# ketanfatania/QMRI-PnP-Recon-POC

Measured on NVIDIA B200. Metric: ADMM slice-iterations/s (224x224x10 slices; step = 120-slice PnP-ADMM recon + T1/T2/PD matching), higher is better.
Workload: dtype f32 (x-update fp32 FFT; denoiser split-bf16 tcgen05, fp32 accumulate; matching fp32)

## Files before the change

### qmri-pnp-recon-poc_b200/csrc/conv_kernels.h

```cpp
#pragma once
#include <stddef.h>
#include <stdint.h>

struct qmri_ctx;

struct ConvParams {
    const float* in;
    const float* w;
    float* out;
    const float* res1;
    const float* res2;
    int S, H, W;
    int Cin, Cout;
    int relu;
    int mode;
    const uint16_t* in_hi = nullptr;
    const uint16_t* in_lo = nullptr;
    uint16_t* out_hi = nullptr;
    uint16_t* out_lo = nullptr;
};

struct HeadTailParams {
    const float* planar_in;
    const float* noise_map;
    float* planar_out;
    float* nhwc;
    const float* w;
    const float* minmax;
    int S, H, W, Cin;
    uint16_t* nhwc_hi = nullptr;
    uint16_t* nhwc_lo = nullptr;
};

enum { TC_CONV3X3 = 0, TC_DOWN2X2 = 1, TC_UP2X2 = 2 };
struct TcConvParams {
    uint16_t* out_hi;
    uint16_t* out_lo;
    const uint16_t* res1_hi;
    const uint16_t* res1_lo;
    const uint16_t* res2_hi;
    const uint16_t* res2_lo;
    int mode;
    int S, H, W;
    int Cin, Cout;
    int BW, BH, tiles_x, tiles_y;
    int relu;
    float* partial;
    int* tickets;
    const void* mapA_hi[4];
    const void* mapA_lo[4];
    const void* mapB_hi;
    const void* mapB_lo;
    const void* mapB_h2;
    const void* mapB_l2;
    const void* mapO_hi;
    const void* mapO_lo;
    const void* mapR_hi;
    const void* mapR_lo;
};

int conv3x3_fp32(qmri_ctx* ctx, const ConvParams& p);
int resample_fp32(qmri_ctx* ctx, const ConvParams& p);
int head_fp32(qmri_ctx* ctx, const HeadTailParams& p);
int tail_fp32(qmri_ctx* ctx, const HeadTailParams& p);
int head_pack_tc(qmri_ctx* ctx, const HeadTailParams& p);
int tail_unpack_tc(qmri_ctx* ctx, const HeadTailParams& p);
int tc_make_act_map(void* out_map, const void* base, int S, int H, int W, int C, int BW, int BH);
int tc_make_down_map(void* out_map, const void* base, int S, int H, int W, int C, int dy, int dx, int BW, int BH);
int tc_make_weight_map(void* out_map, const void* base, int K, int N, int BN);
int tc_tile_shape(int W, int H, int* BW, int* BH);
int tc_block_n(int Cout);
size_t tc_partial_elems(int sm_count);
size_t tc_ticket_count(int sm_count);
int conv_tc(qmri_ctx* ctx, const TcConvParams& p);
int tc_slab_tile_shape(int W, int H, int* BW, int* BH);
void tc_pair_weight_boxes(int Cout, int* rows_main, int* rows_h2);
int conv3x3_tc_pair(qmri_ctx* ctx, const TcConvParams& p);
bool conv64_swap_supported(int W, int H, int Cin, int Cout);
int conv64_swap(qmri_ctx* ctx, const TcConvParams& p, const uint16_t* w_hi, const uint16_t* w_lo);
int normalize_planar(qmri_ctx* ctx, const float* in, float* out, const float* minmax, size_t per_slice, int S, int undo);
```

### qmri-pnp-recon-poc_b200/csrc/conv_tc.cu

```cuda
#include <cuda.h>
#include <cuda_bf16.h>
#include <math.h>
#include <stdlib.h>
#include <string.h>
#include <time.h>
#include <unistd.h>

#include "common.cuh"
#include "conv_kernels.h"

namespace {

constexpr int TC_THREADS = 192;
constexpr int PAIR_THREADS = 224;
constexpr int TC_BM = 128;
constexpr int TC_BK = 64;
constexpr uint32_t A_TILE_BYTES = TC_BM * TC_BK * 2;

template <int BN>
struct TcCfg {
    static constexpr uint32_t B_TILE_BYTES = BN * TC_BK * 2;
    static constexpr uint32_t STAGE_BYTES = 2 * A_TILE_BYTES + 2 * B_TILE_BYTES;
    static constexpr int STAGES = (BN == 64) ? 4 : 3;
    static constexpr uint32_t TMEM_COLS = 2 * BN;
// ... 1794 lines not shown
#pragma unroll
                    for (int i = 0; i < 16; ++i) {
                        const int co = 16 * seg + i;
                        v[i] = tile[co * SW_N + 32 * q + ((lane + co) & 31)];
                    }
                    const size_t o = (((size_t)s * p.H + y) * p.W + x) * 64 + 16 * seg;
                    if (p.res1_hi) {
                        const uint4* gh = reinterpret_cast<const uint4*>(p.res1_hi + o);
                        const uint4* gl = reinterpret_cast<const uint4*>(p.res1_lo + o);
                        add_split8(v, gh[0], gl[0]);
                        add_split8(v + 8, gh[1], gl[1]);
                    }
                    if (p.res2_hi) {
                        const uint4* gh = reinterpret_cast<const uint4*>(p.res2_hi + o);
                        const uint4* gl = reinterpret_cast<const uint4*>(p.res2_lo + o);
                        add_split8(v, gh[0], gl[0]);
                        add_split8(v + 8, gh[1], gl[1]);
                    }
                    store_split16(p.out_hi + o, p.out_lo + o, v, p.relu);
                }
            }
        }
    }
    tc_fence_before();
    __syncthreads();
    if (warp == 1) {
        tc_fence_after();
        asm volatile("tcgen05.dealloc.cta_group::1.sync.aligned.b32 %0, %1;" ::"r"(tmem_base), "r"(512));
    }
}

bool conv64_swap_supported(int W, int H, int Cin, int Cout) { return Cin == 64 && Cout == 64 && W % SW_BW == 0 && H % SW_BH == 0; }
int conv64_swap(qmri_ctx* ctx, const TcConvParams& p, const uint16_t* w_hi, const uint16_t* w_lo) {
    if (!conv64_swap_supported(p.W, p.H, p.Cin, p.Cout)) return qmri_fail(QMRI_EINVAL, "conv64_swap: %d x %d, %d -> %d channels", p.W, p.H, p.Cin, p.Cout);
    if (!p.mapA_hi[0] || !p.mapA_lo[0] || !w_hi || !w_lo) return qmri_fail(QMRI_EINVAL, "conv64_swap: missing tensor map / weights");
    static bool configured_dev[QMRI_MAX_DEV] = {};
    bool& configured = configured_dev[qmri_dev_slot(ctx)];
    if (!configured) {
        QCUDA(cudaFuncSetAttribute(tc_conv64_swap_kernel, cudaFuncAttributeMaxDynamicSharedMemorySize, (int)SW_SMEM));
        configured = true;
    }
    SwapK k;
    k.out_hi = p.out_hi; k.out_lo = p.out_lo;
    k.res1_hi = p.res1_hi; k.res1_lo = p.res1_lo;
    k.res2_hi = p.res2_hi; k.res2_lo = p.res2_lo;
    k.w_hi = w_hi; k.w_lo = w_lo;
    k.S = p.S; k.H = p.H; k.W = p.W;
    k.tiles_x = p.W / SW_BW; k.tiles_y = p.H / SW_BH;
    k.relu = p.relu;
    const int ntiles = k.tiles_x * k.tiles_y * p.S;
    cudaLaunchConfig_t cfg = {};
    cfg.gridDim = dim3(ntiles < ctx->sm_count ? ntiles : ctx->sm_count);
    cfg.blockDim = dim3(TC_THREADS);
    cfg.dynamicSmemBytes = SW_SMEM;
    cfg.stream = ctx->stream;
    cudaLaunchAttribute attr[1];
    attr[0].id = cudaLaunchAttributeProgrammaticStreamSerialization;
    attr[0].val.programmaticStreamSerializationAllowed = tc_pdl_enabled() ? 1 : 0;
    cfg.attrs = attr;
    cfg.numAttrs = 1;
    QCUDA(cudaLaunchKernelEx(&cfg, tc_conv64_swap_kernel, *(const CUtensorMap*)p.mapA_hi[0], *(const CUtensorMap*)p.mapA_lo[0], (const SwapK)k));
    QLAUNCH_CHECK(ctx);
    return QMRI_OK;
}

int conv3x3_tc_pair(qmri_ctx* ctx, const TcConvParams& p) {
    if (p.Cin % TC_BK) return qmri_fail(QMRI_EINVAL, "conv3x3_tc_pair: Cin %% 64");
    if (p.Cout != 64 && p.Cout != 128 && p.Cout % 256) return qmri_fail(QMRI_EINVAL, "conv3x3_tc_pair: Cout %d", p.Cout);
    if (p.BW % 8 || p.BW * p.BH != TC_BM || (p.BH + 2) * p.BW * 128 > (int)PairCfg<256, 0>::A_PLANE)
        return qmri_fail(QMRI_EINVAL, "conv3x3_tc_pair: tile %d x %d not supported", p.BW, p.BH);
    if (!p.mapA_hi[0] || !p.mapA_lo[0] || !p.mapB_hi || !p.mapB_lo || !p.mapB_h2) return qmri_fail(QMRI_EINVAL, "conv3x3_tc_pair: missing tensor map");
    TcK k;
    k.out_hi = p.out_hi; k.out_lo = p.out_lo;
    k.res1_hi = p.res1_hi; k.res1_lo = p.res1_lo;
    k.res2_hi = p.res2_hi; k.res2_lo = p.res2_lo;
    k.partial = p.partial; k.tickets = p.tickets;
    k.S = p.S; k.H = p.H; k.W = p.W; k.Cin = p.Cin; k.Cout = p.Cout;
    k.BW = p.BW; k.BH = p.BH; k.tiles_x = p.tiles_x; k.tiles_y = p.tiles_y;
    k.relu = p.relu; k.nsplit = 1; k.trace = nullptr; k.cluster_splitk = 0; k.dual = 0; k.resw = 0; k.tma_out = 0; k.res_tma = 0; k.l2pf = 0; k.prof = nullptr;
    if (p.Cout == 64) return launch_pair<128, 1>(ctx, p, k);
    if (p.Cout == 128) return launch_pair<256, 1>(ctx, p, k);
    return launch_pair<256, 0>(ctx, p, k);
}
```

### qmri-pnp-recon-poc_b200/csrc/unetres.cu

```cuda
#include <stdlib.h>
#include <string.h>

#include <vector>

#include "common.cuh"
#include "conv_kernels.h"
#include "unetres.h"

static const int NC[4] = {64, 128, 256, 512};

namespace {

struct LayerDesc {
    int kind;
    int cin, cout;
};

std::vector<LayerDesc> layer_table(int in_nc) {
    std::vector<LayerDesc> L;
    L.push_back({3, in_nc, NC[0]});
    for (int lvl = 0; lvl < 3; ++lvl) {
        for (int i = 0; i < 8; ++i) L.push_back({0, NC[lvl], NC[lvl]});
        L.push_back({1, NC[lvl], NC[lvl + 1]});
    }
// ... 80 lines not shown

size_t unetres_weight_count(int in_nc, int layer) {
    auto L = layer_table(in_nc);
    const LayerDesc& d = L[layer];
    int k = (d.kind == 1 || d.kind == 2) ? 4 : 9;
    return (size_t)k * d.cin * d.cout;
}

int unetres_create(qmri_ctx* ctx, int in_nc, const float* const* weights, int n_weights, qmri_net** out) {
    if (!ctx || !weights || !out) return qmri_fail(QMRI_EINVAL, "qmri_unetres_load: null argument");
    if (in_nc != 10 && in_nc != 11)
        return qmri_fail(QMRI_EUNSUPPORTED, "UNetRes in_nc must be 10 (single_level) or 11 (multi_level), got %d", in_nc);
    if (n_weights != 64) return qmri_fail(QMRI_EINVAL, "UNetRes state_dict has 64 weight tensors, got %d", n_weights);
    DevSetter ds(ctx->device);
    qmri_net* net = new qmri_net();
    net->ctx = ctx;
    net->in_nc = in_nc;
    if (const char* e = getenv("QMRI_TC_PAIR")) net->tc_pair = atoi(e);
    auto L = layer_table(in_nc);
    std::vector<float> packed;
    for (int o = 0; o < 2; ++o) {
        net->w[o].assign(64, nullptr);
        for (int l = 0; l < 64; ++l) {
            if (!weights[l]) {
                unetres_free(net);
                return qmri_fail(QMRI_EINVAL, "qmri_unetres_load: weight tensor %d is null", l);
            }
            pack_layer(L[l], weights[l], o, packed);
            int r = dev_alloc(&net->w[o][l], packed.size());
            if (r) {
                unetres_free(net);
                return r;
            }
            cudaError_t e = cudaMemcpy(net->w[o][l], packed.data(), packed.size() * sizeof(float), cudaMemcpyHostToDevice);
            if (e != cudaSuccess) {
                unetres_free(net);
                return qmri_fail(QMRI_ECUDA, "weight upload failed: %s", cudaGetErrorString(e));
            }
        }
        net->wtc_hi[o].assign(64, nullptr);
        net->wtc_lo[o].assign(64, nullptr);
        net->wmap_hi[o].resize(64);
        net->wmap_lo[o].resize(64);
        net->wmapp_hi[o].resize(64);
        net->wmapp_lo[o].resize(64);
        net->wmapp_h2[o].resize(64);
        net->wmapp_l2[o].resize(64);
        std::vector<uint16_t> hi, lo;
        std::vector<float> wpad;
        for (int l = 0; l < 64 && net->tc_available; ++l) {
            LayerDesc dl = L[l];
            const float* wsrc = weights[l];
            if (dl.kind > 2) {
                wpad.assign((size_t)64 * 64 * 9, 0.f);
                for (int co = 0; co < dl.cout; ++co)
                    for (int ci = 0; ci < dl.cin; ++ci)
                        for (int t = 0; t < 9; ++t) wpad[((size_t)co * 64 + ci) * 9 + t] = weights[l][((size_t)co * dl.cin + ci) * 9 + t];
                dl = LayerDesc{0, 64, 64};
                wsrc = wpad.data();
            }
            pack_layer_tc(dl, wsrc, o, hi, lo);
            int r = dev_alloc(&net->wtc_hi[o][l], hi.size()) | dev_alloc(&net->wtc_lo[o][l], lo.size());
            if (r) {
                unetres_free(net);
                return r;
            }
            cudaMemcpy(net->wtc_hi[o][l], hi.data(), hi.size() * 2, cudaMemcpyHostToDevice);
            cudaMemcpy(net->wtc_lo[o][l], lo.data(), lo.size() * 2, cudaMemcpyHostToDevice);
            const int BN = tc_block_n(dl.cout);
            const int K = (dl.kind == 0 ? 9 : dl.kind == 1 ? 4 : 1) * dl.cin;
            const int N = (dl.kind == 2 ? 4 : 1) * dl.cout;
            r = tc_make_weight_map(&net->wmap_hi[o][l], net->wtc_hi[o][l], K, N, BN) |
                tc_make_weight_map(&net->wmap_lo[o][l], net->wtc_lo[o][l], K, N, BN);
            if (!r && dl.kind == 0) {
                int rows_main, rows_h2;
                tc_pair_weight_boxes(dl.cout, &rows_main, &rows_h2);
                r = tc_make_weight_map(&net->wmapp_hi[o][l], net->wtc_hi[o][l], K, N, rows_main) |
                    tc_make_weight_map(&net->wmapp_lo[o][l], net->wtc_lo[o][l], K, N, rows_main) |
                    tc_make_weight_map(&net->wmapp_h2[o][l], net->wtc_hi[o][l], K, N, rows_h2) |
                    tc_make_weight_map(&net->wmapp_l2[o][l], net->wtc_lo[o][l], K, N, rows_h2);
            }
            if (r) net->tc_available = false;
        }
    }
    if (net->tc_available) {
        const size_t np = tc_partial_elems(ctx->sm_count), nt = tc_ticket_count(ctx->sm_count);
        int r = dev_alloc(&net->tc_partial, np) | dev_alloc(&net->tc_tickets, nt);
        if (r) {
            unetres_free(net);
            return r;
        }
        cudaMemset(net->tc_tickets, 0, nt * sizeof(int));
    } else {
        net->precision = 0;
    }
    *out = net;
    return QMRI_OK;
}

void unetres_free(qmri_net* net) {
    if (!net) return;
    DevSetter ds(net->ctx->device);
    for (int o = 0; o < 2; ++o) {
        for (float* p : net->w[o])
            if (p) cudaFree(p);
        for (uint16_t* p : net->wtc_hi[o])
            if (p) cudaFree(p);
        for (uint16_t* p : net->wtc_lo[o])
            if (p) cudaFree(p);
    }
    if (net->ws) cudaFree(net->ws);
    if (net->io) cudaFree(net->io);
    if (net->tc_partial) cudaFree(net->tc_partial);
    if (net->tc_tickets) cudaFree(net->tc_tickets);
    delete net;
}

static size_t level_elems(int lvl, int H, int W) { return (size_t)(H >> lvl) * (W >> lvl) * NC[lvl]; }

int unetres_reserve(qmri_net* net, int S, int H, int W) {
    size_t per_slice = 0;
    for (int l = 0; l < 4; ++l) per_slice += 3 * level_elems(l, H, W);
    const char* env_chunk = getenv("QMRI_NET_CHUNK");
    if (env_chunk && atoi(env_chunk) > 0) net->max_chunk = atoi(env_chunk);
    const int nchunks = (S + net->max_chunk - 1) / net->max_chunk;
    int chunk = nchunks > 0 ? (S + nchunks - 1) / nchunks : S;
    size_t need = per_slice * chunk;
    if (need > net->ws_elems) {
        DevSetter ds(net->ctx->device);
        if (net->ws) cudaFree(net->ws);
        net->ws = nullptr;
        net->ws_elems = 0;
        QCHECK(dev_alloc(&net->ws, need));
        net->ws_elems = need;
    }
    net->chunk = chunk;
    return QMRI_OK;
}

static int forward_chunk(qmri_net* net, const float* in, float* out, const float* minmax, const float* noise_map,
                         int S, int H, int W, int orient) {
    qmri_ctx* ctx = net->ctx;
    float* base = net->ws;
    float *X[4], *A[4], *T[4];
    for (int l = 0; l < 4; ++l) {
        size_t n = level_elems(l, H, W) * S;
        X[l] = base;
        A[l] = base + n;
        T[l] = base + 2 * n;
        base += 3 * n;
    }
    const std::vector<float*>& w = net->w[orient];
    int li = 0;
    HeadTailParams hp = {};
    hp.planar_in = in;
    hp.noise_map = (net->in_nc == 11) ? noise_map : nullptr;
    if (net->in_nc == 11 && !noise_map) return qmri_fail(QMRI_EINVAL, "11-channel denoiser needs a noise map");
    hp.nhwc = X[0];
    hp.w = w[li++];
    hp.minmax = minmax;
    hp.S = S; hp.H = H; hp.W = W; hp.Cin = net->in_nc;
    QCHECK(head_fp32(ctx, hp));

    auto conv = [&](int lvl, const float* src, float* dst, const float* wt, int relu, const float* r1, const float* r2) {
        ConvParams p = {};
        p.in = src; p.w = wt; p.out = dst; p.res1 = r1; p.res2 = r2;
        p.S = S; p.H = H >> lvl; p.W = W >> lvl; p.Cin = NC[lvl]; p.Cout = NC[lvl]; p.relu = relu;
        return conv3x3_fp32(ctx, p);
    };
    auto resblocks = [&](int lvl, const float* src, const float* skip) {
        for (int b = 0; b < 4; ++b) {
            const float* xin = (b == 0) ? src : A[lvl];
            QCHECK(conv(lvl, xin, T[lvl], w[li++], 1, nullptr, nullptr));
            QCHECK(conv(lvl, T[lvl], A[lvl], w[li++], 0, xin, (b == 3) ? skip : nullptr));
        }
        return (int)QMRI_OK;
    };
    for (int lvl = 0; lvl < 3; ++lvl) {
        QCHECK(resblocks(lvl, X[lvl], nullptr));
        ConvParams p = {};
        p.in = A[lvl]; p.w = w[li++]; p.out = X[lvl + 1];
        p.S = S; p.H = H >> lvl; p.W = W >> lvl; p.Cin = NC[lvl]; p.Cout = NC[lvl + 1]; p.mode = 0;
        QCHECK(resample_fp32(ctx, p));
    }
    QCHECK(resblocks(3, X[3], X[3]));
    for (int lvl = 2; lvl >= 0; --lvl) {
        ConvParams p = {};
        p.in = A[lvl + 1]; p.w = w[li++]; p.out = T[lvl];
        p.S = S; p.H = H >> (lvl + 1); p.W = W >> (lvl + 1); p.Cin = NC[lvl + 1]; p.Cout = NC[lvl]; p.mode = 1;
        QCHECK(resample_fp32(ctx, p));
        float* tmp = A[lvl]; A[lvl] = T[lvl]; T[lvl] = tmp;
        for (int b = 0; b < 4; ++b) {
// ... 32 lines not shown
        tc_tile_shape(W >> l, H >> l, &BW, &BH);
        for (int b = 0; b < 3; ++b) {
            QCHECK(tc_make_act_map(&net->amap[b][l][0], hi[b][l], net->chunk, H >> l, W >> l, NC[l], BW, BH));
            QCHECK(tc_make_act_map(&net->amap[b][l][1], lo[b][l], net->chunk, H >> l, W >> l, NC[l], BW, BH));
            int SW, SH;
            tc_slab_tile_shape(W >> l, H >> l, &SW, &SH);
            QCHECK(tc_make_act_map(&net->amap_slab[b][l][0], hi[b][l], net->chunk, H >> l, W >> l, NC[l], SW, SH + 2));
            QCHECK(tc_make_act_map(&net->amap_slab[b][l][1], lo[b][l], net->chunk, H >> l, W >> l, NC[l], SW, SH + 2));
            if (l == 0) {
                QCHECK(tc_make_act_map(&net->amap_tile[b][0], hi[b][0], net->chunk, H, W, NC[0], SW, SH));
                QCHECK(tc_make_act_map(&net->amap_tile[b][1], lo[b][0], net->chunk, H, W, NC[0], SW, SH));
            }
            if (l == 0 && conv64_swap_supported(W, H, NC[0], NC[0])) {
                QCHECK(tc_make_act_map(&net->amap_swap[b][0], hi[b][0], net->chunk, H, W, NC[0], 16, 16));
                QCHECK(tc_make_act_map(&net->amap_swap[b][1], lo[b][0], net->chunk, H, W, NC[0], 16, 16));
            }
            if (l < 3) {
                int DW, DH;
                tc_tile_shape(W >> (l + 1), H >> (l + 1), &DW, &DH);
                for (int tap = 0; tap < 4; ++tap) {
                    QCHECK(tc_make_down_map(&net->amap_down[b][l][tap][0], hi[b][l], net->chunk, H >> l, W >> l, NC[l], tap >> 1, tap & 1, DW, DH));
                    QCHECK(tc_make_down_map(&net->amap_down[b][l][tap][1], lo[b][l], net->chunk, H >> l, W >> l, NC[l], tap >> 1, tap & 1, DW, DH));
                }
            }
        }
    }
    net->amap_ws = net->ws;
    net->amap_chunk = net->chunk;
    net->amap_H = H;
    net->amap_W = W;
    return QMRI_OK;
}

struct LayerProf {
    std::vector<cudaEvent_t> ev;
    std::vector<const char*> names;
    bool on = false;
    void mark(qmri_ctx* ctx, const char* name) {
        if (!on) return;
        cudaEvent_t e;
        cudaEventCreate(&e);
        cudaEventRecord(e, ctx->stream);
        ev.push_back(e);
        names.push_back(name);
    }
    void report(int S) {
        if (!on || ev.empty()) return;
        cudaEventSynchronize(ev.back());
        double tot = 0;
        for (size_t i = 1; i < ev.size(); ++i) {
            float ms = 0;
            cudaEventElapsedTime(&ms, ev[i - 1], ev[i]);
            fprintf(stderr, "[qmri profile] S=%d %-10s %8.1f us\n", S, names[i], ms * 1e3);
            tot += ms;
        }
        fprintf(stderr, "[qmri profile] S=%d total %8.1f us\n", S, tot * 1e3);
        for (auto e : ev) cudaEventDestroy(e);
        ev.clear();
        names.clear();
    }
};

static int forward_chunk_tc(qmri_net* net, const float* in, float* out, const float* minmax, const float* noise_map,
                            int S, int H, int W, int orient) {
    qmri_ctx* ctx = net->ctx;
    LayerProf prof;
    prof.on = getenv("QMRI_PROFILE") != nullptr;
    prof.mark(ctx, "start");
    uint16_t *hi[3][4], *lo[3][4];
    tc_buffers(net, H, W, hi, lo);
    enum { BX = 0, BA = 1, BT = 2 };
    int roleA[4] = {BA, BA, BA, BA}, roleT[4] = {BT, BT, BT, BT};
    const std::vector<float*>& w = net->w[orient];
    int li = 0;
    if (net->in_nc == 11 && !noise_map) return qmri_fail(QMRI_EINVAL, "11-channel denoiser needs a noise map");
    HeadTailParams hp = {};
    hp.planar_in = in;
    hp.noise_map = (net->in_nc == 11) ? noise_map : nullptr;
    hp.nhwc_hi = hi[BX][0];
    hp.nhwc_lo = lo[BX][0];
    hp.w = w[li++];
    hp.minmax = minmax;
    hp.S = S; hp.H = H; hp.W = W; hp.Cin = net->in_nc;
    const char* ht_env = getenv("QMRI_TC_HEADTAIL");
    const bool ht_tc = !(ht_env && atoi(ht_env) == 0);
    if (!ht_tc) {
        QCHECK(head_fp32(ctx, hp));
        prof.mark(ctx, "head");
    }

    auto tiles = [&](TcConvParams& p) {
        tc_tile_shape(p.W, p.H, &p.BW, &p.BH);
        p.tiles_x = (p.W + p.BW - 1) / p.BW;
        p.tiles_y = (p.H + p.BH - 1) / p.BH;
        p.partial = net->tc_partial;
        p.tickets = net->tc_tickets;
    };
    auto conv = [&](int lvl, int src, int dst, int layer, int relu, int r1, int r2) {
        TcConvParams p = {};
        p.mode = TC_CONV3X3;
        p.out_hi = hi[dst][lvl]; p.out_lo = lo[dst][lvl];
        p.res1_hi = r1 >= 0 ? hi[r1][lvl] : nullptr; p.res1_lo = r1 >= 0 ? lo[r1][lvl] : nullptr;
        p.res2_hi = r2 >= 0 ? hi[r2][lvl] : nullptr; p.res2_lo = r2 >= 0 ? lo[r2][lvl] : nullptr;
        p.S = S; p.H = H >> lvl; p.W = W >> lvl; p.Cin = NC[lvl]; p.Cout = NC[lvl];
        p.relu = relu;
        tiles(p);
        {
            const char* sw_env = getenv("QMRI_TC_SWAP");
            const bool sw_on = sw_env ? atoi(sw_env) != 0 : net->tc_swap != 0;
            if (lvl == 0 && sw_on && conv64_swap_supported(p.W, p.H, p.Cin, p.Cout) && (p.W / 16) * (p.H / 14) * S >= ctx->sm_count) {
                p.mapA_hi[0] = &net->amap_swap[src][0]; p.mapA_lo[0] = &net->amap_swap[src][1];
                return conv64_swap(ctx, p, net->wtc_hi[orient][layer], net->wtc_lo[orient][layer]);
            }
        }
        int SW, SH;
        tc_slab_tile_shape(p.W, p.H, &SW, &SH);
        const int pair_groups = ((((p.W + SW - 1) / SW) * ((p.H + SH - 1) / SH) * S + 1) / 2) * (NC[lvl] >= 256 ? NC[lvl] / 256 : 1);
        if (((net->tc_pair >> lvl) & 1) && (pair_groups >= ctx->sm_count / 2 || (net->tc_pair & 16))) {
            p.BW = SW;
            p.BH = SH;
            p.tiles_x = (p.W + p.BW - 1) / p.BW;
            p.tiles_y = (p.H + p.BH - 1) / p.BH;
            p.mapA_hi[0] = &net->amap_slab[src][lvl][0]; p.mapA_lo[0] = &net->amap_slab[src][lvl][1];
            p.mapB_hi = &net->wmapp_hi[orient][layer]; p.mapB_lo = &net->wmapp_lo[orient][layer];
            p.mapB_h2 = &net->wmapp_h2[orient][layer];
            p.mapB_l2 = &net->wmapp_l2[orient][layer];
            if (lvl == 0) {
                p.mapO_hi = &net->amap_tile[dst][0]; p.mapO_lo = &net->amap_tile[dst][1];
                if (r1 >= 0) {
                    p.mapR_hi = &net->amap_tile[r1][0]; p.mapR_lo = &net->amap_tile[r1][1];
                }
            }
            return conv3x3_tc_pair(ctx, p);
        }
        p.mapA_hi[0] = &net->amap[src][lvl][0]; p.mapA_lo[0] = &net->amap[src][lvl][1];
        p.mapB_hi = &net->wmap_hi[orient][layer]; p.mapB_lo = &net->wmap_lo[orient][layer];
        return conv_tc(ctx, p);
    };
    auto resample = [&](int lvl_in, int src, int lvl_out, int dst, int layer, int up) {
        TcConvParams p = {};
        p.mode = up ? TC_UP2X2 : TC_DOWN2X2;
        p.out_hi = hi[dst][lvl_out]; p.out_lo = lo[dst][lvl_out];
        const int lm = up ? lvl_in : lvl_out;
        p.S = S; p.H = H >> lm; p.W = W >> lm; p.Cin = NC[lvl_in]; p.Cout = NC[lvl_out];
        tiles(p);
        if (up) {
            p.mapA_hi[0] = &net->amap[src][lvl_in][0]; p.mapA_lo[0] = &net->amap[src][lvl_in][1];
        } else {
            for (int tap = 0; tap < 4; ++tap) {
                p.mapA_hi[tap] = &net->amap_down[src][lvl_in][tap][0];
                p.mapA_lo[tap] = &net->amap_down[src][lvl_in][tap][1];
            }
        }
        p.mapB_hi = &net->wmap_hi[orient][layer]; p.mapB_lo = &net->wmap_lo[orient][layer];
        return conv_tc(ctx, p);
    };
    if (ht_tc) {
        hp.nhwc_hi = hi[BT][0];
        hp.nhwc_lo = lo[BT][0];
        QCHECK(head_pack_tc(ctx, hp));
        QCHECK(conv(0, BT, BX, 0, 0, -1, -1));
        prof.mark(ctx, "head");
    }
    for (int lvl = 0; lvl < 3; ++lvl) {
        for (int b = 0; b < 4; ++b) {
            int xin = (b == 0) ? BX : roleA[lvl];
            QCHECK(conv(lvl, xin, roleT[lvl], li, 1, -1, -1)); ++li;
            prof.mark(ctx, lvl == 0 ? "conv L0" : lvl == 1 ? "conv L1" : "conv L2");
            QCHECK(conv(lvl, roleT[lvl], roleA[lvl], li, 0, xin, -1)); ++li;
            prof.mark(ctx, lvl == 0 ? "conv L0 r" : lvl == 1 ? "conv L1 r" : "conv L2 r");
        }
        QCHECK(resample(lvl, roleA[lvl], lvl + 1, BX, li, 0)); ++li;
        prof.mark(ctx, "down");
    }
    for (int b = 0; b < 4; ++b) {
        int xin = (b == 0) ? BX : roleA[3];
        QCHECK(conv(3, xin, roleT[3], li, 1, -1, -1)); ++li;
        prof.mark(ctx, "conv L3");
        QCHECK(conv(3, roleT[3], roleA[3], li, 0, xin, (b == 3) ? BX : -1)); ++li;
        prof.mark(ctx, "conv L3 r");
    }
    for (int lvl = 2; lvl >= 0; --lvl) {
        QCHECK(resample(lvl + 1, roleA[lvl + 1], lvl, roleT[lvl], li, 1)); ++li;
        prof.mark(ctx, "up");
        int tmp = roleA[lvl]; roleA[lvl] = roleT[lvl]; roleT[lvl] = tmp;
        for (int b = 0; b < 4; ++b) {
            QCHECK(conv(lvl, roleA[lvl], roleT[lvl], li, 1, -1, -1)); ++li;
            prof.mark(ctx, lvl == 0 ? "conv L0" : lvl == 1 ? "conv L1" : "conv L2");
            QCHECK(conv(lvl, roleT[lvl], roleA[lvl], li, 0, roleA[lvl], (b == 3) ? BX : -1)); ++li;
            prof.mark(ctx, lvl == 0 ? "conv L0 r" : lvl == 1 ? "conv L1 r" : "conv L2 r");
        }
    }
    HeadTailParams tp = {};
    tp.nhwc_hi = hi[roleA[0]][0];
    tp.nhwc_lo = lo[roleA[0]][0];
    tp.planar_out = out;
    tp.w = w[li++];
    tp.minmax = minmax;
    tp.S = S; tp.H = H; tp.W = W; tp.Cin = 64;
    if (ht_tc) {
        QCHECK(conv(0, roleA[0], roleT[0], li - 1, 0, -1, -1));
        tp.nhwc_hi = hi[roleT[0]][0];
        tp.nhwc_lo = lo[roleT[0]][0];
        QCHECK(tail_unpack_tc(ctx, tp));
    } else {
        QCHECK(tail_fp32(ctx, tp));
    }
    prof.mark(ctx, "tail");
    prof.report(S);
    return QMRI_OK;
}

int unetres_forward_dev(qmri_net* net, const float* in, float* out, const float* minmax, const float* noise_map,
                        int S, int H, int W, int orient) {
    if (!net || !in || !out) return qmri_fail(QMRI_EINVAL, "unetres forward: null argument");
    if (S <= 0) return QMRI_OK;
    if (H % 8 || W % 8 || H < 8 || W < 8) return qmri_fail(QMRI_EINVAL, "UNetRes needs H, W multiples of 8 (got %d x %d)", H, W);
    if (net->precision == 1 && !net->tc_available)
        return qmri_fail(QMRI_EUNSUPPORTED, "tensor mode unavailable: cuTensorMapEncodeTiled could not be resolved");
    DevSetter ds(net->ctx->device);
    QCHECK(unetres_reserve(net, S, H, W));
    if (net->precision == 1) QCHECK(build_act_maps(net, H, W));
    const int Cpl = (net->in_nc == 11) ? 10 : net->in_nc;
    for (int s0 = 0; s0 < S; s0 += net->chunk) {
        int n = (S - s0 < net->chunk) ? S - s0 : net->chunk;
        if (net->precision == 1)
            QCHECK(forward_chunk_tc(net, in + (size_t)s0 * Cpl * H * W, out + (size_t)s0 * 10 * H * W,
                                    minmax ? minmax + 2 * s0 : nullptr, noise_map, n, H, W, orient));
        else
            QCHECK(forward_chunk(net, in + (size_t)s0 * Cpl * H * W, out + (size_t)s0 * 10 * H * W,
                                 minmax ? minmax + 2 * s0 : nullptr, noise_map, n, H, W, orient));
    }
    return QMRI_OK;
}

double unetres_flops(int in_nc, int S, int H, int W) {
    auto L = layer_table(in_nc);
    double f = 0;
    int lvl = 0;
    for (const auto& d : L) {
        double px;
        if (d.kind == 3 || d.kind == 4) px = (double)H * W;
        else if (d.kind == 0) {
            for (lvl = 0; lvl < 4; ++lvl)
                if (NC[lvl] == d.cin) break;
            px = (double)(H >> lvl) * (W >> lvl);
        } else if (d.kind == 1) {
            for (lvl = 0; lvl < 4; ++lvl)
                if (NC[lvl] == d.cout) break;
            px = (double)(H >> lvl) * (W >> lvl);
            f += 2.0 * px * 4 * d.cin * d.cout;
            continue;
        } else {
            for (lvl = 0; lvl < 4; ++lvl)
                if (NC[lvl] == d.cin) break;
            px = (double)(H >> lvl) * (W >> lvl);
            f += 2.0 * px * 4 * d.cin * d.cout;
            continue;
        }
        f += 2.0 * px * 9 * d.cin * d.cout;
    }
    return f * S;
}
```

### qmri-pnp-recon-poc_b200/csrc/unetres.h

```cpp
#pragma once
#include <stddef.h>
#include <stdint.h>

#include <vector>

struct qmri_ctx;

struct alignas(64) TMap {
    unsigned char bytes[128];
};

struct qmri_net {
    qmri_ctx* ctx = nullptr;
    int in_nc = 10;
    int precision = 1;
    bool tc_available = true;
    std::vector<float*> w[2];
    float* ws = nullptr;
    size_t ws_elems = 0;
    int max_chunk = 128;
    int chunk = 0;
    float* io = nullptr;
    size_t io_elems = 0;
    std::vector<uint16_t*> wtc_hi[2], wtc_lo[2];
    std::vector<TMap> wmap_hi[2], wmap_lo[2];
    TMap amap[3][4][2];
    TMap amap_slab[3][4][2];
    TMap amap_tile[3][2];
    TMap amap_swap[3][2];
    int tc_swap = 0;
    std::vector<TMap> wmapp_hi[2], wmapp_lo[2], wmapp_h2[2], wmapp_l2[2];
    int tc_pair = 15;
    TMap amap_down[3][3][4][2];
    float* tc_partial = nullptr;
    int* tc_tickets = nullptr;
    const float* amap_ws = nullptr;
    int amap_chunk = 0, amap_H = 0, amap_W = 0;
};

int unetres_create(qmri_ctx* ctx, int in_nc, const float* const* weights, int n_weights, qmri_net** out);
void unetres_free(qmri_net* net);
int unetres_reserve(qmri_net* net, int S, int H, int W);
int unetres_forward_dev(qmri_net* net, const float* in, float* out, const float* minmax, const float* noise_map,
                        int S, int H, int W, int orient);
double unetres_flops(int in_nc, int S, int H, int W);
size_t unetres_weight_count(int in_nc, int layer);
```

Baseline: 1688.

## Add dedicated tcgen05 head and tail conv kernels replacing padded-channel path

Adds a fused head kernel that reads planar input, normalizes, splits into bf16 hi/lo, builds im2col tiles with only the real 10-11 channels, and runs the 3x3 conv on tcgen05 with the NHWC hi/lo output written directly. It also adds a tail kernel that does the 64->10 conv with a narrow N=32 weight map and writes denormalized planar fp32 output straight from TMEM. Together these replace the old pack-then-full-conv head and conv-then-unpack tail, which padded the channels to 64 and spent extra passes and launches. This becomes the default path, while the old padded path stays selectable through an environment value. The cost is a lot of new hand-written warp-specialized code whose correctness depends on the custom weight layouts.

```diff
diff --git a/qmri-pnp-recon-poc_b200/csrc/conv_kernels.h b/qmri-pnp-recon-poc_b200/csrc/conv_kernels.h
--- a/qmri-pnp-recon-poc_b200/csrc/conv_kernels.h
+++ b/qmri-pnp-recon-poc_b200/csrc/conv_kernels.h
@@ -65,6 +65,11 @@
 int tail_fp32(qmri_ctx* ctx, const HeadTailParams& p);
 int head_pack_tc(qmri_ctx* ctx, const HeadTailParams& p);
 int tail_unpack_tc(qmri_ctx* ctx, const HeadTailParams& p);
+size_t tc_head_weight_elems();
+void tc_head_weight_image(const uint16_t* w_hi, const uint16_t* w_lo, int Cin, uint16_t* img);
+void tc_tail_weight_rows(const uint16_t* w_hi, const uint16_t* w_lo, int Cout, uint16_t* rows);
+int head_tc(qmri_ctx* ctx, const HeadTailParams& p, const uint16_t* w_img);
+int tail_tc(qmri_ctx* ctx, const HeadTailParams& p, const void* map_a_hi, const void* map_a_lo, const void* map_w, int BW, int BH);
 int tc_make_act_map(void* out_map, const void* base, int S, int H, int W, int C, int BW, int BH);
 int tc_make_down_map(void* out_map, const void* base, int S, int H, int W, int C, int dy, int dx, int BW, int BH);
 int tc_make_weight_map(void* out_map, const void* base, int K, int N, int BN);
diff --git a/qmri-pnp-recon-poc_b200/csrc/conv_tc.cu b/qmri-pnp-recon-poc_b200/csrc/conv_tc.cu
--- a/qmri-pnp-recon-poc_b200/csrc/conv_tc.cu
+++ b/qmri-pnp-recon-poc_b200/csrc/conv_tc.cu
@@ -1900,3 +1900,480 @@
     if (p.Cout == 128) return launch_pair<256, 1>(ctx, p, k);
     return launch_pair<256, 0>(ctx, p, k);
 }
+
+namespace {
+
+constexpr uint32_t HD_BLK = TC_BM * 128;
+constexpr uint32_t HD_STAGE = 5 * HD_BLK;
+constexpr int HD_STAGES = 2;
+constexpr uint32_t HD_WBLK = 64 * 128;
+constexpr uint32_t HD_WBYTES = 5 * HD_WBLK;
+constexpr int HD_THREADS = 288;
+constexpr uint32_t HD_PATCH = 34 * 6 * 64;
+constexpr uint32_t HD_EPI = 4 * 32 * 64;
+constexpr size_t HD_SMEM = (size_t)HD_STAGES * HD_STAGE + HD_WBYTES + HD_PATCH + HD_EPI + 1024 + 256;
+
+constexpr int TL_STAGES = 4;
+constexpr uint32_t TL_SLAB_MAX = 20480;
+constexpr uint32_t TL_WTAP = 32 * 128;
+constexpr uint32_t TL_WBYTES = 9 * TL_WTAP;
+constexpr size_t TL_SMEM = (size_t)TL_STAGES * 2 * TL_SLAB_MAX + TL_WBYTES + 1024 + 256;
+
+struct HtK {
+    const float* in;
+    const float* noise;
+    const float* minmax;
+    float* out;
+    uint16_t *out_hi, *out_lo;
+    const uint4* w;
+    int S, H, W, BW, BH, tiles_x, tiles_y;
+};
+
+struct TlMaps {
+    CUtensorMap a_hi, a_lo, w;
+};
+
+__host__ __device__ __forceinline__ int hd_block(int t, int plane) { return t < 8 ? plane * 2 + t / 4 : 4; }
+__host__ __device__ __forceinline__ int hd_kstep(int t, int plane) { return t < 8 ? t % 4 : plane; }
+
+__global__ void __launch_bounds__(HD_THREADS, 1) tc_head_kernel(const HtK p) {
+    extern __shared__ unsigned char tc_smem_raw[];
+    const uint32_t raw = smem_u32(tc_smem_raw);
+    unsigned char* smem = tc_smem_raw + ((1024u - (raw & 1023u)) & 1023u);
+    unsigned char* sW = smem + (size_t)HD_STAGES * HD_STAGE;
+    unsigned char* sP = sW + HD_WBYTES;
+    unsigned char* sE = sP + HD_PATCH;
+    uint64_t* bars = reinterpret_cast<uint64_t*>(sE + HD_EPI);
+    uint64_t* full = bars;
+    uint64_t* empty = bars + 2;
+    uint64_t* tfull = bars + 4;
+    uint64_t* tempty = bars + 6;
+    uint32_t* tmem_slot = reinterpret_cast<uint32_t*>(bars + 8);
+
+    const int warp = __shfl_sync(0xffffffffu, threadIdx.x >> 5, 0), lane = threadIdx.x & 31;
+    const int tiles_xy = p.tiles_x * p.tiles_y;
+    const int ntiles = tiles_xy * p.S;
+    const size_t HW = (size_t)p.H * p.W;
+    if (threadIdx.x == 0) {
+        for (int i = 0; i < 2; ++i) {
+            mbar_init(&full[i], 128);
+            mbar_init(&empty[i], 1);
+            mbar_init(&tfull[i], 1);
+            mbar_init(&tempty[i], 4);
+        }
+        asm volatile("fence.mbarrier_init.release.cluster;" ::: "memory");
+    }
+    if (warp == 8) {
+        asm volatile("tcgen05.alloc.cta_group::1.sync.aligned.shared::cta.b32 [%0], %1;" ::"r"(smem_u32(tmem_slot)), "r"(128));
+        asm volatile("tcgen05.relinquish_alloc_permit.cta_group::1.sync.aligned;" ::);
+    }
+    for (uint32_t i = threadIdx.x; i < HD_WBYTES / 16; i += HD_THREADS) reinterpret_cast<uint4*>(sW)[i] = __ldg(p.w + i);
+    asm volatile("fence.proxy.async.shared::cta;" ::: "memory");
+    pdl_launch_dependents();
+    tc_fence_before();
+    __syncthreads();
+    tc_fence_after();
+    const uint32_t tmem_base = __shfl_sync(0xffffffffu, *tmem_slot, 0);
+    pdl_wait();
+
+    if (warp < 4) {
+        const int row = threadIdx.x;
+        const int r7 = row & 7;
+        const int PW = p.BW + 2, npatch = PW * (p.BH + 2);
+        const uint32_t patch = smem_u32(sP);
+        float raw[2][11];
+        auto load_patch = [&](int t) {
+            const int txy = t % tiles_xy, s = t / tiles_xy;
+            const int x0 = (txy % p.tiles_x) * p.BW - 1, y0 = (txy / p.tiles_x) * p.BH - 1;
+            const float* src = p.in + (size_t)s * 10 * HW;
+#pragma unroll
+            for (int k = 0; k < 2; ++k) {
+                const int i = row + 128 * k;
+                const int yy = y0 + i / PW, xx = x0 + i % PW;
+                const bool in_img = i < npatch && yy >= 0 && yy < p.H && xx >= 0 && xx < p.W;
+                const size_t off = in_img ? (size_t)yy * p.W + xx : 0;
+#pragma unroll
+                for (int c = 0; c < 10; ++c) raw[k][c] = in_img ? __ldg(src + c * HW + off) : 0.f;
+                raw[k][10] = (in_img && p.noise) ? __ldg(p.noise + off) : 0.f;
+            }
+        };
+        if (blockIdx.x < ntiles) load_patch(blockIdx.x);
+        int it = 0;
+        for (int t = blockIdx.x; t < ntiles; t += gridDim.x, ++it) {
+            const int st = it & 1;
+            const uint32_t ph = (it >> 1) & 1;
+            const int txy = t % tiles_xy, s = t / tiles_xy;
+            const int x0 = (txy % p.tiles_x) * p.BW - 1, y0 = (txy / p.tiles_x) * p.BH - 1;
+            float mn = 0.f, inv = 1.f;
+            if (p.minmax) {
+                mn = p.minmax[2 * s];
+                inv = 1.0f / (p.minmax[2 * s + 1] - mn);
+            }
+            asm volatile("bar.sync 1, 128;" ::: "memory");
+#pragma unroll
+            for (int k = 0; k < 2; ++k) {
+                const int i = row + 128 * k;
+                if (i < npatch) {
+                    const int yy = y0 + i / PW, xx = x0 + i % PW;
+                    const bool in_img = yy >= 0 && yy < p.H && xx >= 0 && xx < p.W;
+                    float v[12];
+#pragma unroll
+                    for (int c = 0; c < 10; ++c) v[c] = in_img ? (raw[k][c] - mn) * inv : 0.f;
+                    v[10] = raw[k][10];
+                    v[11] = 0.f;
+                    uint32_t hi[8], lo[8];
+#pragma unroll
+                    for (int j = 0; j < 8; ++j) {
+                        const float a = j < 6 ? v[2 * j] : 0.f, b = j < 6 ? v[2 * j + 1] : 0.f;
+                        hi[j] = pack_bf16(a, b);
+                        float ha, hb;
+                        unpack_bf16(hi[j], ha, hb);
+                        lo[j] = pack_bf16(a - ha, b - hb);
+                    }
+                    const uint32_t a = patch + (uint32_t)i * 64;
+                    const uint32_t sw = (uint32_t)((i >> 1) & 3);
+                    asm volatile("st.shared.v4.b32 [%0], {%1, %2, %3, %4};" ::"r"(a + ((0 ^ sw) << 4)), "r"(hi[0]), "r"(hi[1]), "r"(hi[2]), "r"(hi[3]) : "memory");
+                    asm volatile("st.shared.v4.b32 [%0], {%1, %2, %3, %4};" ::"r"(a + ((1 ^ sw) << 4)), "r"(hi[4]), "r"(hi[5]), "r"(hi[6]), "r"(hi[7]) : "memory");
+                    asm volatile("st.shared.v4.b32 [%0], {%1, %2, %3, %4};" ::"r"(a + ((2 ^ sw) << 4)), "r"(lo[0]), "r"(lo[1]), "r"(lo[2]), "r"(lo[3]) : "memory");
+                    asm volatile("st.shared.v4.b32 [%0], {%1, %2, %3, %4};" ::"r"(a + ((3 ^ sw) << 4)), "r"(lo[4]), "r"(lo[5]), "r"(lo[6]), "r"(lo[7]) : "memory");
+                }
+            }
+            if (t + (int)gridDim.x < ntiles) load_patch(t + gridDim.x);
+            asm volatile("bar.sync 1, 128;" ::: "memory");
+            mbar_wait(&empty[st], ph ^ 1);
+            const uint32_t rbase = smem_u32(smem + (size_t)st * HD_STAGE) + (uint32_t)row * 128;
+            const int pr = (row / p.BW) * PW + row % p.BW;
+#pragma unroll
+            for (int tap = 0; tap < 9; ++tap) {
+                const int pi = pr + (tap / 3) * PW + tap % 3;
+                const uint32_t src = patch + (uint32_t)pi * 64, sw = (uint32_t)((pi >> 1) & 3);
+#pragma unroll
+                for (int plane = 0; plane < 2; ++plane) {
+                    uint4 q0, q1;
+                    asm volatile("ld.shared.v4.b32 {%0, %1, %2, %3}, [%4];" : "=r"(q0.x), "=r"(q0.y), "=r"(q0.z), "=r"(q0.w) : "r"(src + (((2 * plane) ^ sw) << 4)) : "memory");
+                    asm volatile("ld.shared.v4.b32 {%0, %1, %2, %3}, [%4];" : "=r"(q1.x), "=r"(q1.y), "=r"(q1.z), "=r"(q1.w) : "r"(src + (((2 * plane + 1) ^ sw) << 4)) : "memory");
+                    const uint32_t rb = rbase + (uint32_t)hd_block(tap, plane) * HD_BLK;
+                    const int c0 = 2 * hd_kstep(tap, plane);
+                    asm volatile("st.shared.v4.b32 [%0], {%1, %2, %3, %4};" ::"r"(rb + (uint32_t)((c0 ^ r7) << 4)), "r"(q0.x), "r"(q0.y), "r"(q0.z), "r"(q0.w) : "memory");
+                    asm volatile("st.shared.v4.b32 [%0], {%1, %2, %3, %4};" ::"r"(rb + (uint32_t)(((c0 + 1) ^ r7) << 4)), "r"(q1.x), "r"(q1.y), "r"(q1.z), "r"(q1.w) : "memory");
+                }
+            }
+            asm volatile("fence.proxy.async.shared::cta;" ::: "memory");
+            mbar_arrive(&full[st]);
+        }
+    } else if (warp < 8) {
+        const int lg = warp & 3;
+        const uint32_t stage = smem_u32(sE) + (uint32_t)lg * 2048;
+        int it = 0;
+        for (int t = blockIdx.x; t < ntiles; t += gridDim.x, ++it) {
+            const int ab = it & 1;
+            const uint32_t aphase = (it >> 1) & 1;
+            const int txy = t % tiles_xy, s = t / tiles_xy;
+            mbar_wait(&tfull[ab], aphase);
+            tc_fence_after();
+            const uint32_t taddr = tmem_base + ((uint32_t)(lg * 32) << 16) + (uint32_t)(ab * 64);
+            const int q4 = lane & 3;
+            size_t po[4];
+            bool pok[4];
+#pragma unroll
+            for (int k = 0; k < 4; ++k) {
+                const int pr = lg * 32 + (lane >> 2) + 8 * k;
+                const int px = (txy % p.tiles_x) * p.BW + pr % p.BW, py = (txy / p.tiles_x) * p.BH + pr / p.BW;
+                pok[k] = px < p.W && py < p.H;
+                po[k] = (((size_t)s * p.H + py) * p.W + px) * 64 + 8 * q4;
+            }
+#pragma unroll
+            for (int c0 = 0; c0 < 64; c0 += 32) {
+                uint32_t acc[2][16];
+                tc_ld16(taddr + c0, acc[0]);
+                tc_ld16(taddr + c0 + 16, acc[1]);
+                tc_wait_ld();
+                uint32_t ph[16], pl[16];
+#pragma unroll
+                for (int j = 0; j < 16; ++j) {
+                    const float a = __uint_as_float(acc[j / 8][2 * (j % 8)]), b = __uint_as_float(acc[j / 8][2 * (j % 8) + 1]);
+                    ph[j] = pack_bf16(a, b);
+                    float ha, hb;
+                    unpack_bf16(ph[j], ha, hb);
+                    pl[j] = pack_bf16(a - ha, b - hb);
+                }
+#pragma unroll
+                for (int plane = 0; plane < 2; ++plane) {
+                    const uint32_t* w = plane ? pl : ph;
+                    uint16_t* out = plane ? p.out_lo : p.out_hi;
+#pragma unroll
+                    for (int j = 0; j < 4; ++j)
+                        asm volatile("st.shared.v4.b32 [%0], {%1, %2, %3, %4};" ::"r"(stage + (uint32_t)lane * 64 + (uint32_t)((j ^ ((lane >> 1) & 3)) << 4)),
+                                     "r"(w[4 * j]), "r"(w[4 * j + 1]), "r"(w[4 * j + 2]), "r"(w[4 * j + 3]) : "memory");
+                    __syncwarp();
+#pragma unroll
+                    for (int k = 0; k < 4; ++k) {
+                        const int pr = (lane >> 2) + 8 * k;
+                        uint4 v;
+                        asm volatile("ld.shared.v4.b32 {%0, %1, %2, %3}, [%4];" : "=r"(v.x), "=r"(v.y), "=r"(v.z), "=r"(v.w)
+                                     : "r"(stage + (uint32_t)pr * 64 + (uint32_t)((q4 ^ ((pr >> 1) & 3)) << 4)) : "memory");
+                        if (pok[k]) *reinterpret_cast<uint4*>(out + po[k] + c0) = v;
+                    }
+                    __syncwarp();
+                }
+            }
+            tc_fence_before();
+            __syncwarp();
+            if (lane == 0) mbar_arrive(&tempty[ab]);
+        }
+    } else {
+        const uint32_t idesc = (1u << 4) | (1u << 7) | (1u << 10) | ((uint32_t)(64 >> 3) << 17) | ((uint32_t)(TC_BM >> 4) << 24);
+        const uint32_t wb = smem_u32(sW);
+        int it = 0;
+        for (int t = blockIdx.x; t < ntiles; t += gridDim.x, ++it) {
+            const int st = it & 1;
+            const uint32_t ph = (it >> 1) & 1;
+            mbar_wait(&tempty[st], ph ^ 1);
+            mbar_wait(&full[st], ph);
+            tc_fence_after();
+            const uint32_t tmem_d = tmem_base + (uint32_t)(st * 64);
+            const uint32_t ab = smem_u32(smem + (size_t)st * HD_STAGE);
+#pragma unroll
+            for (int tap = 0; tap < 9; ++tap) {
+                const uint64_t a_hi = umma_desc(ab + hd_block(tap, 0) * HD_BLK) + 2 * hd_kstep(tap, 0);
+                const uint64_t a_lo = umma_desc(ab + hd_block(tap, 1) * HD_BLK) + 2 * hd_kstep(tap, 1);
+                const uint64_t b_hi = umma_desc(wb + hd_block(tap, 0) * HD_WBLK) + 2 * hd_kstep(tap, 0);
+                const uint64_t b_lo = umma_desc(wb + hd_block(tap, 1) * HD_WBLK) + 2 * hd_kstep(tap, 1);
+                tc_mma_elect(tmem_d, a_hi, b_hi, idesc, tap ? 1u : 0u);
+                tc_mma_elect(tmem_d, a_hi, b_lo, idesc, 1u);
+                tc_mma_elect(tmem_d, a_lo, b_hi, idesc, 1u);
+            }
+            tc_commit_elect(&empty[st]);
+            tc_commit_elect(&tfull[st]);
+        }
+    }
+    tc_fence_before();
+    __syncthreads();
+    if (warp == 8) {
+        tc_fence_after();
+        asm volatile("tcgen05.dealloc.cta_group::1.sync.aligned.b32 %0, %1;" ::"r"(tmem_base), "r"(128));
+    }
+}
+
+__global__ void __launch_bounds__(TC_THREADS, 1) tc_tail_kernel(const __grid_constant__ TlMaps maps, const HtK p) {
+    extern __shared__ unsigned char tc_smem_raw[];
+    const uint32_t raw = smem_u32(tc_smem_raw);
+    unsigned char* smem = tc_smem_raw + ((1024u - (raw & 1023u)) & 1023u);
+    unsigned char* sA = smem + TL_WBYTES;
+    uint64_t* bars = reinterpret_cast<uint64_t*>(sA + (size_t)TL_STAGES * 2 * TL_SLAB_MAX);
+    uint64_t* full = bars;
+    uint64_t* empty = bars + TL_STAGES;
+    uint64_t* tfull = bars + 2 * TL_STAGES;
+    uint64_t* tempty = bars + 2 * TL_STAGES + 2;
+    uint64_t* wfull = bars + 2 * TL_STAGES + 4;
+    uint32_t* tmem_slot = reinterpret_cast<uint32_t*>(bars + 2 * TL_STAGES + 5);
+
+    const int warp = __shfl_sync(0xffffffffu, threadIdx.x >> 5, 0), lane = threadIdx.x & 31;
+    const int tiles_xy = p.tiles_x * p.tiles_y;
+    const int ntiles = tiles_xy * p.S;
+    const uint32_t slab_bytes = (uint32_t)((p.BH + 2) * p.BW * 128);
+    const uint32_t dy_bytes = (uint32_t)(p.BW * 128);
+    if (threadIdx.x == 0) {
+        for (int i = 0; i < TL_STAGES; ++i) {
+            mbar_init(&full[i], 1);
+            mbar_init(&empty[i], 1);
+        }
+        for (int i = 0; i < 2; ++i) {
+            mbar_init(&tfull[i], 1);
+            mbar_init(&tempty[i], 4);
+        }
+        mbar_init(wfull, 1);
+        asm volatile("fence.mbarrier_init.release.cluster;" ::: "memory");
+        tma_prefetch_desc(&maps.a_hi);
+        tma_prefetch_desc(&maps.a_lo);
+        tma_prefetch_desc(&maps.w);
+    }
+    if (warp == 1) {
+        asm volatile("tcgen05.alloc.cta_group::1.sync.aligned.shared::cta.b32 [%0], %1;" ::"r"(smem_u32(tmem_slot)), "r"(64));
+        asm volatile("tcgen05.relinquish_alloc_permit.cta_group::1.sync.aligned;" ::);
+    }
+    pdl_launch_dependents();
+    tc_fence_before();
+    __syncthreads();
+    tc_fence_after();
+    const uint32_t tmem_base = __shfl_sync(0xffffffffu, *tmem_slot, 0);
+    pdl_wait();
+
+    if (warp == 0) {
+        if (lane == 0) {
+            mbar_expect_tx(wfull, TL_WBYTES);
+            for (int tap = 0; tap < 9; ++tap) tma_load_2d(smem + tap * TL_WTAP, &maps.w, wfull, tap * 64, 0);
+            int stage = 0;
+            uint32_t phase = 0;
+            for (int t = blockIdx.x; t < ntiles; t += gridDim.x) {
+                const int txy = t % tiles_xy, s = t / tiles_xy;
+                const int x0 = (txy % p.tiles_x) * p.BW, y0 = (txy / p.tiles_x) * p.BH;
+                for (int dxi = 0; dxi < 3; ++dxi) {
+                    mbar_wait(&empty[stage], phase ^ 1);
+                    unsigned char* st = sA + (size_t)stage * 2 * TL_SLAB_MAX;
+                    mbar_expect_tx(&full[stage], 2 * slab_bytes);
+                    tma_load_4d(st, &maps.a_hi, &full[stage], 0, x0 + dxi - 1, y0 - 1, s);
+                    tma_load_4d(st + slab_bytes, &maps.a_lo, &full[stage], 0, x0 + dxi - 1, y0 - 1, s);
+                    if (++stage == TL_STAGES) {
+                        stage = 0;
+                        phase ^= 1;
+                    }
+                }
+            }
+        }
+    } else if (warp == 1) {
+        const uint32_t idesc0 = (1u << 4) | (1u << 7) | (1u << 10) | ((uint32_t)(TC_BM >> 4) << 24);
+        const uint32_t idesc32 = idesc0 | ((uint32_t)(32 >> 3) << 17), idesc16 = idesc0 | ((uint32_t)(16 >> 3) << 17);
+        const uint32_t wb = smem_u32(smem);
+        int stage = 0;
+        uint32_t phase = 0;
+        int it = 0;
+        if (blockIdx.x < ntiles) {
+            mbar_wait(wfull, 0);
+            tc_fence_after();
+        }
+        for (int t = blockIdx.x; t < ntiles; t += gridDim.x, ++it) {
+            const int ab = it & 1;
+            const uint32_t aphase = (it >> 1) & 1;
+            mbar_wait(&tempty[ab], aphase ^ 1);
+            tc_fence_after();
+            const uint32_t tmem_d = tmem_base + (uint32_t)(ab * 32);
+            for (int dxi = 0; dxi < 3; ++dxi) {
+                mbar_wait(&full[stage], phase);
+                tc_fence_after();
+                const uint32_t sa = smem_u32(sA + (size_t)stage * 2 * TL_SLAB_MAX);
+#pragma unroll
+                for (int dyi = 0; dyi < 3; ++dyi) {
+                    const uint64_t a_hi = umma_desc(sa + dyi * dy_bytes), a_lo = umma_desc(sa + slab_bytes + dyi * dy_bytes);
+                    const uint64_t b = umma_desc(wb + (uint32_t)(dyi * 3 + dxi) * TL_WTAP);
+#pragma unroll
+                    for (int k = 0; k < TC_BK / 16; ++k) {
+                        const uint64_t ko = (uint64_t)(k * 2);
+                        tc_mma_elect(tmem_d, a_hi + ko, b + ko, idesc32, (dxi | dyi | k) ? 1u : 0u);
+                        tc_mma_elect(tmem_d, a_lo + ko, b + ko, idesc16, 1u);
+                    }
+                }
+                tc_commit_elect(&empty[stage]);
+                if (++stage == TL_STAGES) {
+                    stage = 0;
+                    phase ^= 1;
+                }
+            }
+            tc_commit_elect(&tfull[ab]);
+        }
+    } else {
+        const int lg = warp & 3;
+        const int row = lg * 32 + lane;
+        const size_t HW = (size_t)p.H * p.W;
+        int it = 0;
+        for (int t = blockIdx.x; t < ntiles; t += gridDim.x, ++it) {
+            const int ab = it & 1;
+            const uint32_t aphase = (it >> 1) & 1;
+            const int txy = t % tiles_xy, s = t / tiles_xy;
+            const int x = (txy % p.tiles_x) * p.BW + row % p.BW;
+            const int y = (txy / p.tiles_x) * p.BH + row / p.BW;
+            float mn = 0.f, rg = 1.f;
+            if (p.minmax) {
+                mn = p.minmax[2 * s];
+                rg = p.minmax[2 * s + 1] - mn;
+            }
+            mbar_wait(&tfull[ab], aphase);
+            tc_fence_after();
+            const uint32_t taddr = tmem_base + ((uint32_t)(lg * 32) << 16) + (uint32_t)(ab * 32);
+            uint32_t acc[2][16];
+            tc_ld16(taddr, acc[0]);
+            tc_ld16(taddr + 16, acc[1]);
+            tc_wait_ld();
+            tc_fence_before();
+            __syncwarp();
+            if (lane == 0) mbar_arrive(&tempty[ab]);
+            if (x < p.W && y < p.H) {
+                float* o = p.out + (size_t)s * 10 * HW + (size_t)y * p.W + x;
+#pragma unroll
+                for (int c = 0; c < 10; ++c) o[c * HW] = (__uint_as_float(acc[0][c]) + __uint_as_float(acc[1][c])) * rg + mn;
+            }
+        }
+    }
+    tc_fence_before();
+    __syncthreads();
+    if (warp == 1) {
+        tc_fence_after();
+        asm volatile("tcgen05.dealloc.cta_group::1.sync.aligned.b32 %0, %1;" ::"r"(tmem_base), "r"(64));
+    }
+}
+
+template <typename Kern>
+int launch_headtail(qmri_ctx* ctx, Kern kern, size_t smem_bytes, int threads, int ntiles, bool* configured, const TlMaps* maps, const HtK& k) {
+    if (!*configured) {
+        QCUDA(cudaFuncSetAttribute(kern, cudaFuncAttributeMaxDynamicSharedMemorySize, (int)smem_bytes));
+        *configured = true;
+    }
+    cudaLaunchConfig_t cfg = {};
+    cfg.gridDim = dim3(ntiles < ctx->sm_count ? ntiles : ctx->sm_count);
+    cfg.blockDim = dim3(threads);
+    cfg.dynamicSmemBytes = smem_bytes;
+    cfg.stream = ctx->stream;
+    cudaLaunchAttribute attr[1];
+    attr[0].id = cudaLaunchAttributeProgrammaticStreamSerialization;
+    attr[0].val.programmaticStreamSerializationAllowed = tc_pdl_enabled() ? 1 : 0;
+    cfg.attrs = attr;
+    cfg.numAttrs = 1;
+    if (maps) QCUDA(cudaLaunchKernelEx(&cfg, tc_tail_kernel, *maps, k));
+    else QCUDA(cudaLaunchKernelEx(&cfg, tc_head_kernel, k));
+    QLAUNCH_CHECK(ctx);
+    return QMRI_OK;
+}
+
+}
+
+size_t tc_head_weight_elems() { return HD_WBYTES / 2; }
+
+void tc_head_weight_image(const uint16_t* w_hi, const uint16_t* w_lo, int Cin, uint16_t* img) {
+    memset(img, 0, HD_WBYTES);
+    for (int r = 0; r < 64; ++r)
+        for (int tap = 0; tap < 9; ++tap)
+            for (int plane = 0; plane < 2; ++plane) {
+                const uint16_t* w = plane ? w_lo : w_hi;
+                for (int ci = 0; ci < Cin; ++ci) {
+                    const int j = 2 * hd_kstep(tap, plane) + ci / 8;
+                    img[(size_t)hd_block(tap, plane) * (HD_WBLK / 2) + r * 64 + ((j ^ (r & 7)) * 8) + ci % 8] = w[((size_t)r * 9 + tap) * Cin + ci];
+                }
+            }
+}
+
+void tc_tail_weight_rows(const uint16_t* w_hi, const uint16_t* w_lo, int Cout, uint16_t* rows) {
+    memset(rows, 0, (size_t)32 * 576 * 2);
+    memcpy(rows, w_hi, (size_t)Cout * 576 * 2);
+    memcpy(rows + (size_t)16 * 576, w_lo, (size_t)Cout * 576 * 2);
+}
+
+int head_tc(qmri_ctx* ctx, const HeadTailParams& p, const uint16_t* w_img) {
+    if ((p.Cin != 10 && p.Cin != 11) || (p.Cin == 11) != (p.noise_map != nullptr) || !p.nhwc_hi || !p.nhwc_lo || !w_img)
+        return qmri_fail(QMRI_EINVAL, "head_tc: Cin %d / missing noise map, planes or weights", p.Cin);
+    static bool configured_dev[QMRI_MAX_DEV] = {};
+    HtK k = {};
+    k.in = p.planar_in; k.noise = p.noise_map; k.minmax = p.minmax;
+    k.out_hi = p.nhwc_hi; k.out_lo = p.nhwc_lo;
+    k.w = reinterpret_cast<const uint4*>(w_img);
+    k.S = p.S; k.H = p.H; k.W = p.W;
+    tc_tile_shape(p.W, p.H, &k.BW, &k.BH);
+    k.tiles_x = (p.W + k.BW - 1) / k.BW;
+    k.tiles_y = (p.H + k.BH - 1) / k.BH;
+    return launch_headtail(ctx, tc_head_kernel, HD_SMEM, HD_THREADS, k.tiles_x * k.tiles_y * p.S, &configured_dev[qmri_dev_slot(ctx)], nullptr, k);
+}
+
+int tail_tc(qmri_ctx* ctx, const HeadTailParams& p, const void* map_a_hi, const void* map_a_lo, const void* map_w, int BW, int BH) {
+    if (!p.planar_out || !map_a_hi || !map_a_lo || !map_w) return qmri_fail(QMRI_EINVAL, "tail_tc: missing output or tensor map");
+    if (BW % 8 || BW * BH != TC_BM || (uint32_t)((BH + 2) * BW * 128) > TL_SLAB_MAX) return qmri_fail(QMRI_EINVAL, "tail_tc: tile %d x %d not supported", BW, BH);
+    static bool configured_dev[QMRI_MAX_DEV] = {};
+    TlMaps maps;
+    maps.a_hi = *(const CUtensorMap*)map_a_hi;
+    maps.a_lo = *(const CUtensorMap*)map_a_lo;
+    maps.w = *(const CUtensorMap*)map_w;
+    HtK k = {};
+    k.out = p.planar_out; k.minmax = p.minmax;
+    k.S = p.S; k.H = p.H; k.W = p.W; k.BW = BW; k.BH = BH;
+    k.tiles_x = (p.W + BW - 1) / BW;
+    k.tiles_y = (p.H + BH - 1) / BH;
+    return launch_headtail(ctx, tc_tail_kernel, TL_SMEM, TC_THREADS, k.tiles_x * k.tiles_y * p.S, &configured_dev[qmri_dev_slot(ctx)], &maps, k);
+}
diff --git a/qmri-pnp-recon-poc_b200/csrc/unetres.cu b/qmri-pnp-recon-poc_b200/csrc/unetres.cu
--- a/qmri-pnp-recon-poc_b200/csrc/unetres.cu
+++ b/qmri-pnp-recon-poc_b200/csrc/unetres.cu
@@ -186,6 +186,21 @@
             }
             if (r) net->tc_available = false;
         }
+        if (net->tc_available) {
+            std::vector<uint16_t> img(tc_head_weight_elems()), rows((size_t)32 * 576);
+            pack_layer_tc(LayerDesc{0, in_nc, 64}, weights[0], o, hi, lo);
+            tc_head_weight_image(hi.data(), lo.data(), in_nc, img.data());
+            pack_layer_tc(LayerDesc{0, 64, 10}, weights[63], o, hi, lo);
+            tc_tail_weight_rows(hi.data(), lo.data(), 10, rows.data());
+            int r = dev_alloc(&net->wht_head[o], img.size()) | dev_alloc(&net->wht_tail[o], rows.size());
+            if (r) {
+                unetres_free(net);
+                return r;
+            }
+            cudaMemcpy(net->wht_head[o], img.data(), img.size() * 2, cudaMemcpyHostToDevice);
+            cudaMemcpy(net->wht_tail[o], rows.data(), rows.size() * 2, cudaMemcpyHostToDevice);
+            if (tc_make_weight_map(&net->wmap_tail[o], net->wht_tail[o], 576, 32, 32)) net->tc_available = false;
+        }
     }
     if (net->tc_available) {
         const size_t np = tc_partial_elems(ctx->sm_count), nt = tc_ticket_count(ctx->sm_count);
@@ -212,6 +227,8 @@
             if (p) cudaFree(p);
         for (uint16_t* p : net->wtc_lo[o])
             if (p) cudaFree(p);
+        if (net->wht_head[o]) cudaFree(net->wht_head[o]);
+        if (net->wht_tail[o]) cudaFree(net->wht_tail[o]);
     }
     if (net->ws) cudaFree(net->ws);
     if (net->io) cudaFree(net->io);
@@ -410,9 +427,10 @@
     hp.w = w[li++];
     hp.minmax = minmax;
     hp.S = S; hp.H = H; hp.W = W; hp.Cin = net->in_nc;
+    enum { HT_REAL, HT_PAD, HT_FP32 };
     const char* ht_env = getenv("QMRI_TC_HEADTAIL");
-    const bool ht_tc = !(ht_env && atoi(ht_env) == 0);
-    if (!ht_tc) {
+    const int ht = !ht_env ? HT_REAL : strcmp(ht_env, "pad") == 0 ? HT_PAD : atoi(ht_env) == 0 ? HT_FP32 : HT_REAL;
+    if (ht == HT_FP32) {
         QCHECK(head_fp32(ctx, hp));
         prof.mark(ctx, "head");
     }
@@ -483,7 +501,10 @@
         p.mapB_hi = &net->wmap_hi[orient][layer]; p.mapB_lo = &net->wmap_lo[orient][layer];
         return conv_tc(ctx, p);
     };
-    if (ht_tc) {
+    if (ht == HT_REAL) {
+        QCHECK(head_tc(ctx, hp, net->wht_head[orient]));
+        prof.mark(ctx, "head");
+    } else if (ht == HT_PAD) {
         hp.nhwc_hi = hi[BT][0];
         hp.nhwc_lo = lo[BT][0];
         QCHECK(head_pack_tc(ctx, hp));
@@ -526,7 +547,11 @@
     tp.w = w[li++];
     tp.minmax = minmax;
     tp.S = S; tp.H = H; tp.W = W; tp.Cin = 64;
-    if (ht_tc) {
+    if (ht == HT_REAL) {
+        int SW, SH;
+        tc_slab_tile_shape(W, H, &SW, &SH);
+        QCHECK(tail_tc(ctx, tp, &net->amap_slab[roleA[0]][0][0], &net->amap_slab[roleA[0]][0][1], &net->wmap_tail[orient], SW, SH));
+    } else if (ht == HT_PAD) {
         QCHECK(conv(0, roleA[0], roleT[0], li - 1, 0, -1, -1));
         tp.nhwc_hi = hi[roleT[0]][0];
         tp.nhwc_lo = lo[roleT[0]][0];
diff --git a/qmri-pnp-recon-poc_b200/csrc/unetres.h b/qmri-pnp-recon-poc_b200/csrc/unetres.h
--- a/qmri-pnp-recon-poc_b200/csrc/unetres.h
+++ b/qmri-pnp-recon-poc_b200/csrc/unetres.h
@@ -24,6 +24,9 @@
     size_t io_elems = 0;
     std::vector<uint16_t*> wtc_hi[2], wtc_lo[2];
     std::vector<TMap> wmap_hi[2], wmap_lo[2];
+    uint16_t* wht_head[2] = {nullptr, nullptr};
+    uint16_t* wht_tail[2] = {nullptr, nullptr};
+    TMap wmap_tail[2];
     TMap amap[3][4][2];
     TMap amap_slab[3][4][2];
     TMap amap_tile[3][2];
```

New measurement: 1716, median of 6. +1.7%, better.
